# CoHDI/composable-resource-operator

Hardware: NVIDIA H100
Metric: composed-GPU probes/sec (higher is better)
Workload: dtype u64

## Files before the change

__graft_entry__.py:

```python
from __future__ import annotations

import importlib
import os
import subprocess
import sys

ROOT = os.path.dirname(os.path.abspath(__file__))
PKG = os.path.join(ROOT, "composable-resource-operator_b200")
CSRC = os.path.join(PKG, "csrc")
ORACLE = os.path.join(ROOT, "oracle")

NVCC_FLAGS = ["-gencode", "arch=compute_90a,code=sm_90a", "-O3", "-std=c++17", "-lineinfo",
              "-Xcompiler", "-fPIC"]
SOURCES = ["kernels.cu", "probe.cu", "sweeps.cu", "locate.cu", "hbm_scan.cu", "host_link.cu", "compute_probe.cu", "fullbox.cu", "c_api.cu", "harness.cu", "cluster.cu", "gojson.cpp", "identity.cpp", "reconcile.cpp", "detach.cpp",
           "fabric.cpp", "provider.cpp", "nodes.cpp", "gpus.cpp", "gpus_local.cpp", "gotypes.cpp", "env.cpp", "inventory.cpp", "nvml_ops.cpp", "pcilink.cpp",
           "compute.cpp"]


def _newer(target: str, deps) -> bool:
    if not os.path.exists(target):
        return True
    t = os.path.getmtime(target)
    return any(os.path.getmtime(d) > t for d in deps)


def _nvcc() -> str:
    for cand in (os.environ.get("NVCC"), "/usr/local/cuda/bin/nvcc", "nvcc"):
        if cand and (os.path.isabs(cand) and os.path.exists(cand) or not os.path.isabs(cand)):
            return cand
    return "nvcc"


def build_oracle() -> None:
    oso = os.path.join(ORACLE, "liboracle.so")
    osrc = os.path.join(ORACLE, "cro_oracle.c")
    if _newer(oso, [osrc]):
        subprocess.check_call(["gcc", "-O2", "-shared", "-fPIC", "-Wno-format-truncation", "-o", oso, osrc, "-lpthread"])
# ... 91 lines not shown
```

composable-resource-operator_b200/csrc/env.cpp:

```cpp
#include "env.hpp"

#include <cstdlib>
#include <cstring>

namespace cro {
namespace env {

namespace {
const Knob kKnobs[] = {
    {"CRO_FILL_WAVES", 1, 1024, 64, 0, "CTA waves of the fill kernel"},
    {"CRO_READ_WAVES", 1, 1024, 1, 0, "CTA waves of the LDG read kernels"},
    {"CRO_COPY_WAVES", 1, 1024, 128, 0, "CTA waves of the LDG copy kernel"},
    {"CRO_TMA_READ_TILE", 1024, 114688, 32768, 16, "bytes per TMA bulk load of the read ring"},
    {"CRO_TMA_READ_STAGES", 2, 16, 4, 0, "ring depth of the read kernel"},
    {"CRO_TMA_READ_THREADS", 64, 1024, 160, 32, "1 producer warp + consumer warps"},
    {"CRO_TMA_READ_CHUNK", 1, 4096, 1, 0, "tiles claimed per atomic"},
    {"CRO_TMA_READ_HINT", 0, 1, 0, 0, "1 = L2 evict_first on the bulk loads"},
    {"CRO_TMA_READ_DYN", 0, 1, 1, 0, "1 = dynamic tile claims"},
    {"CRO_TMA_READ_WAVES", 1, 64, 1, 0, "CTAs per SM slot"},
    {"CRO_TMA_COPY_TILE", 1024, 114688, 32768, 16, "bytes per TMA bulk copy of the copy ring"},
    {"CRO_TMA_COPY_STAGES", 2, 16, 4, 0, "ring depth of the copy kernel"},
    {"CRO_TMA_COPY_CHUNK", 1, 4096, 1, 0, "tiles claimed per atomic"},
    {"CRO_TMA_COPY_HINT", 0, 7, 0, 0, "bit0 evict_first loads, bit1 evict_first stores, bit2 evict_last stores"},
    {"CRO_TMA_COPY_DYN", 0, 1, 1, 0, "1 = dynamic tile claims"},
    {"CRO_TMA_COPY_WAVES", 1, 64, 1, 0, "CTAs per SM slot"},
    {"CRO_FUSED_TILE", 1024, 114688, 32768, 16, "bytes per tile of the checksumming copy"},
    {"CRO_FUSED_STAGES", 2, 16, 4, 0, "ring depth of the checksumming copy"},
    {"CRO_FUSED_CHUNK", 1, 4096, 1, 0, "tiles claimed per atomic"},
    {"CRO_FUSED_THREADS", 64, 1024, 160, 32, "1 producer warp + consumer warps of the checksumming copy"},
    {"CRO_READ_VARIANT", 0, 3, 0, 0, "CRO_READ_* forced for every sweep (0 = by size)"},
    {"CRO_COPY_VARIANT", 0, 3, 0, 0, "CRO_COPY_* forced (0 = checksumming TMA copy)"},
    {"CRO_USE_GRAPH", 0, 1, 1, 0, "replay the probe as one CUDA graph"},
    {"CRO_EXPECT_OVERLAP", 0, 1, 1, 0, "closed-form generator on a side stream under the copy sweeps"},
    {"CRO_EXPECT_CTAS", 1, 8, 1, 0, "CTAs per SM of the closed-form generator (it must leave room for the copy's CTA)"},
    {"CRO_CARVEOUT_FILL", 0, 1, 1, 0, "the fill kernel asks for the largest shared memory too (it runs beside a generator in cro_probe_all)"},
    {"CRO_P2P_UNIDIR", 0, 1, 0, 0, "measurement only: one direction per NVLink pair"},
    {"CRO_P2P_READ_VARIANT", 1, 3, 2, 0, "kernel of the NVLink read leg"},
    {"CRO_P2P_WRITE_VARIANT", 1, 3, 3, 0, "kernel of the NVLink push leg"},
    {"CRO_NVTX", 0, 1, 1, 0, "NVTX ranges around the probe phases"},
    {"CRO_HELPER_TIMEOUT_MS", 100, 600000, 30000, 0, "deadline of the out-of-process probe helper"},
};
constexpr int kN = (int)(sizeof kKnobs / sizeof kKnobs[0]);

int index_of(const char* name) {
    for (int i = 0; i < kN; ++i)
        if (strcmp(kKnobs[i].name, name) == 0) return i;
    return -1;
}
}

const Knob* table(int* n_out) {
    if (n_out) *n_out = kN;
// ... 58 lines not shown
```

composable-resource-operator_b200/csrc/fullbox.cu:

```cuda
#include <dlfcn.h>

#include "probe_internal.hpp"

namespace cro {

int upload_chase_table(cro_ctx* c, const std::vector<uint32_t>& perm, unsigned long long** table) {
    std::vector<unsigned long long> wide(perm.begin(), perm.end());
    CU_TRY(c, cudaMalloc(table, (size_t)kChaseSlots * 128));
    CU_TRY(c, cudaMemset(*table, 0, (size_t)kChaseSlots * 128));
    CU_TRY(c, cudaMemcpy2D(*table, 128, wide.data(), 8, 8, kChaseSlots, cudaMemcpyHostToDevice));
    CU_TRY(c, cudaStreamSynchronize(0));
    return CRO_OK;
}

namespace {

std::vector<std::vector<std::pair<int, int>>> one_factorisation(int n) {
    std::vector<std::vector<std::pair<int, int>>> rounds;
    if (n < 2) return rounds;
    const int m = (n % 2 == 0) ? n : n + 1;
    for (int r = 0; r < m - 1; ++r) {
        std::vector<std::pair<int, int>> pairs;
        auto add = [&](int a, int b) { if (a < n && b < n) pairs.push_back({a, b}); };
        add(m - 1, r);
// ... 179 lines not shown
    auto pair_ok = [&](int a, int b) { return a < 8 && b < 8 && c->devs[(size_t)a]->tmpl.p2p_access[b]; };
    auto push_bytes = [&](const Device* a, const Device* b) {
        return std::min<uint64_t>(std::min<uint64_t>(o.p2p_bytes, a->sweep_bytes), b->sweep_bytes);
    };
    if (p2p) {
        Range nv(c, "cro.probe_all.nvlink");
        for (size_t r = 0; r < rounds.size(); ++r) {
            std::vector<std::pair<int, int>> directed;
            for (const auto& p : rounds[r]) {
                directed.push_back({p.first, p.second});
                if (!unidir) directed.push_back({p.second, p.first});
            }
            for (const auto& pr : directed) {
                Device* a = c->devs[(size_t)pr.first].get();
                Device* b = c->devs[(size_t)pr.second].get();
                if (!pair_ok(pr.first, pr.second)) continue;
                CU_TRY(c, cudaSetDevice(a->ordinal));
                CU_TRY(c, cudaStreamWaitEvent(a->stream, b->ev_hbm_done, 0));
                if (r > 0) CU_TRY(c, cudaStreamWaitEvent(a->stream, b->ev_reread_done[r - 1], 0));
                CU_TRY(c, launch_read(a->plan, rvp, b->region, std::min<uint64_t>(o.p2p_bytes, b->sweep_bytes), imm_params(a),
                                      a->scratch, &a->d_out[kSlotP2P0 + 3 * pr.second], a->stream));
                c->launches++;
                if (push) {
                    CU_TRY(c, launch_copy(a->plan, wvp, b->region + b->sweep_bytes, a->region, push_bytes(a, b), imm_params(a),
                                          a->scratch, &a->d_out[kSlotP2P0 + 3 * pr.second + 1], a->stream));
                    c->launches++;
                }
                CU_TRY(c, cudaEventRecord(a->ev_push_done[r], a->stream));
            }
            for (const auto& pr : directed) {
                Device* a = c->devs[(size_t)pr.first].get();
                Device* b = c->devs[(size_t)pr.second].get();
                if (!pair_ok(pr.first, pr.second)) continue;
                CU_TRY(c, cudaSetDevice(b->ordinal));
                if (push) {
                    b->half_known[1] = false;
                    CU_TRY(c, cudaStreamWaitEvent(b->stream, a->ev_push_done[r], 0));
                    CU_TRY(c, launch_read(b->plan, resolve_read_variant(CRO_READ_AUTO, push_bytes(a, b), c->knobs), b->region + b->sweep_bytes,
                                          push_bytes(a, b), imm_params(b), b->scratch, &b->d_out[kSlotP2P0 + 3 * pr.first + 2], b->stream));
                    c->launches++;
                }
                CU_TRY(c, cudaEventRecord(b->ev_reread_done[r], b->stream));
            }
            if (unidir)
                for (const auto& p : rounds[r]) {
                    Device* b = c->devs[(size_t)p.second].get();
                    CU_TRY(c, cudaSetDevice(b->ordinal));
// ... 194 lines not shown
```

composable-resource-operator_b200/csrc/kernels.cu:

```cuda
#include "kernels.cuh"

#include <cuda_bf16.h>
#include <cuda_fp8.h>

#include <algorithm>
#include <cstdio>
#include <cstdlib>
#include <type_traits>

namespace cro {

__device__ __forceinline__ unsigned long long globaltimer_ns() {
    unsigned long long t;
    asm volatile("mov.u64 %0, %%globaltimer;" : "=l"(t));
    return t;
}

__device__ __forceinline__ uint4 ldg_stream(const uint4* p) {
    uint4 r;
    asm volatile("ld.global.nc.L1::no_allocate.v4.u32 {%0,%1,%2,%3}, [%4];"
                 : "=r"(r.x), "=r"(r.y), "=r"(r.z), "=r"(r.w)
                 : "l"(p));
    return r;
}

__device__ __forceinline__ uint64_t l2_policy_evict_first() {
    uint64_t p;
    asm volatile("createpolicy.fractional.L2::evict_first.b64 %0, 1.0;" : "=l"(p));
    return p;
}
__device__ __forceinline__ uint64_t l2_policy_evict_last() {
    uint64_t p;
    asm volatile("createpolicy.fractional.L2::evict_last.b64 %0, 1.0;" : "=l"(p));
    return p;
}

template <int STRIDE>
__device__ __forceinline__ void ldg128_x8(const void* p, unsigned long long (&a)[8],
                                          unsigned long long (&b)[8]) {
// ... 14 lines not shown
}
template <int STRIDE>
__device__ __forceinline__ void ldg256_x4(const void* p, uint64_t policy, unsigned long long (&w)[16]) {
    asm volatile(
        "ld.global.nc.L1::no_allocate.L2::cache_hint.v2.u64 {%0,%1}, [%16], %23;\n"
        "ld.global.nc.L1::no_allocate.L2::cache_hint.v2.u64 {%2,%3}, [%16+16], %23;\n"
        "ld.global.nc.L1::no_allocate.L2::cache_hint.v2.u64 {%4,%5}, [%16+%17], %23;\n"
        "ld.global.nc.L1::no_allocate.L2::cache_hint.v2.u64 {%6,%7}, [%16+%20], %23;\n"
        "ld.global.nc.L1::no_allocate.L2::cache_hint.v2.u64 {%8,%9}, [%16+%18], %23;\n"
        "ld.global.nc.L1::no_allocate.L2::cache_hint.v2.u64 {%10,%11}, [%16+%21], %23;\n"
        "ld.global.nc.L1::no_allocate.L2::cache_hint.v2.u64 {%12,%13}, [%16+%19], %23;\n"
        "ld.global.nc.L1::no_allocate.L2::cache_hint.v2.u64 {%14,%15}, [%16+%22], %23;\n"
        : "=l"(w[0]), "=l"(w[1]), "=l"(w[2]), "=l"(w[3]), "=l"(w[4]), "=l"(w[5]), "=l"(w[6]),
          "=l"(w[7]), "=l"(w[8]), "=l"(w[9]), "=l"(w[10]), "=l"(w[11]), "=l"(w[12]), "=l"(w[13]),
          "=l"(w[14]), "=l"(w[15])
        : "l"(p), "n"(STRIDE), "n"(2 * STRIDE), "n"(3 * STRIDE), "n"(STRIDE + 16), "n"(2 * STRIDE + 16),
          "n"(3 * STRIDE + 16), "l"(policy));
}

__device__ __forceinline__ void stg_stream(uint4* p, const uint4& v) {
    asm volatile("st.global.L1::no_allocate.v4.u32 [%0], {%1,%2,%3,%4};" ::"l"(p), "r"(v.x),
                 "r"(v.y), "r"(v.z), "r"(v.w)
                 : "memory");
}

__device__ __forceinline__ unsigned long long lo64(const uint4& v) {
    return (unsigned long long)v.x | ((unsigned long long)v.y << 32);
}
__device__ __forceinline__ unsigned long long hi64(const uint4& v) {
    return (unsigned long long)v.z | ((unsigned long long)v.w << 32);
}

__device__ __forceinline__ uint32_t smem_u32(const void* p) {
    return (uint32_t)__cvta_generic_to_shared(p);
}

__device__ __forceinline__ void mbar_init(uint64_t* bar, uint32_t count) {
    asm volatile("mbarrier.init.shared::cta.b64 [%0], %1;" ::"r"(smem_u32(bar)), "r"(count));
}
__device__ __forceinline__ void mbar_fence_init() {
    asm volatile("fence.mbarrier_init.release.cluster;" ::: "memory");
}
__device__ __forceinline__ void mbar_expect_tx(uint64_t* bar, uint32_t bytes) {
    asm volatile("mbarrier.arrive.expect_tx.shared::cta.b64 _, [%0], %1;" ::"r"(smem_u32(bar)),
                 "r"(bytes)
                 : "memory");
}
__device__ __forceinline__ void mbar_arrive(uint64_t* bar) {
    asm volatile("mbarrier.arrive.shared::cta.b64 _, [%0];" ::"r"(smem_u32(bar)) : "memory");
}
__device__ __forceinline__ void mbar_wait(uint64_t* bar, uint32_t parity) {
    asm volatile(
        "{\n"
        ".reg .pred p;\n"
        "WAIT_%=:\n"
        "mbarrier.try_wait.parity.shared::cta.b64 p, [%0], %1;\n"
        "@p bra DONE_%=;\n"
        "bra WAIT_%=;\n"
        "DONE_%=:\n"
        "}\n" ::"r"(smem_u32(bar)),
        "r"(parity)
        : "memory");
}
__device__ __forceinline__ void tma_load_1d(void* smem_dst, const void* gsrc, uint32_t bytes,
                                            uint64_t* bar) {
    asm volatile(
        "cp.async.bulk.shared::cluster.global.mbarrier::complete_tx::bytes [%0], [%1], %2, [%3];" ::
            "r"(smem_u32(smem_dst)),
        "l"(gsrc), "r"(bytes), "r"(smem_u32(bar))
        : "memory");
}
__device__ __forceinline__ void tma_store_1d(void* gdst, const void* smem_src, uint32_t bytes) {
    asm volatile("cp.async.bulk.global.shared::cta.bulk_group [%0], [%1], %2;" ::"l"(gdst),
                 "r"(smem_u32(smem_src)), "r"(bytes)
                 : "memory");
}
__device__ __forceinline__ void tma_load_1d_hint(void* smem_dst, const void* gsrc, uint32_t bytes,
                                                 uint64_t* bar, uint64_t policy) {
    asm volatile(
        "cp.async.bulk.shared::cluster.global.mbarrier::complete_tx::bytes.L2::cache_hint [%0], [%1], %2, [%3], %4;" ::
            "r"(smem_u32(smem_dst)),
        "l"(gsrc), "r"(bytes), "r"(smem_u32(bar)), "l"(policy)
        : "memory");
}
__device__ __forceinline__ void tma_store_1d_hint(void* gdst, const void* smem_src, uint32_t bytes,
                                                  uint64_t policy) {
    asm volatile("cp.async.bulk.global.shared::cta.bulk_group.L2::cache_hint [%0], [%1], %2, %3;" ::"l"(gdst),
                 "r"(smem_u32(smem_src)), "r"(bytes), "l"(policy)
                 : "memory");
}
__device__ __forceinline__ void tma_commit() {
    asm volatile("cp.async.bulk.commit_group;" ::: "memory");
}
template <int N>
__device__ __forceinline__ void tma_wait_read() {
    asm volatile("cp.async.bulk.wait_group.read %0;" ::"n"(N) : "memory");
}
__device__ __forceinline__ void tma_wait_all() {
    asm volatile("cp.async.bulk.wait_group 0;" ::: "memory");
}

struct Acc {
    unsigned long long x0 = 0, x1 = 0, s = 0, w = 0, d = 0;
};
__device__ __forceinline__ void fold2(Acc& A, unsigned long long a, unsigned long long b,
                                      unsigned long long m ) {
    const unsigned long long c = a + b;
    A.x0 ^= a;
    A.x1 ^= b;
    A.s += c;
    A.w += c * m;
    A.d += b;
}
__device__ __forceinline__ unsigned long long acc_x(const Acc& A) { return A.x0 ^ A.x1; }
__device__ __forceinline__ unsigned long long acc_w(const Acc& A) { return A.w + 2ull * A.d; }

__device__ __forceinline__ void publish(unsigned long long x, unsigned long long s, unsigned long long w,
                                        unsigned long long t_start, const SweepScratch sc,
                                        SweepOut* out, const ProbeParams& imm, const ProbeParams* pp,
                                        unsigned long long n_words) {
    __shared__ unsigned long long sx[32], ss[32], sw[32];
    __shared__ bool is_last;
#pragma unroll
    for (int o = 16; o > 0; o >>= 1) {
        x ^= __shfl_xor_sync(0xffffffffu, x, o);
        s += __shfl_xor_sync(0xffffffffu, s, o);
        w += __shfl_xor_sync(0xffffffffu, w, o);
    }
    const int warp = threadIdx.x >> 5, lane = threadIdx.x & 31;
    const int nwarps = (blockDim.x + 31) >> 5;
    if (lane == 0) { sx[warp] = x; ss[warp] = s; sw[warp] = w; }
    __syncthreads();
    if (warp == 0) {
        x = lane < nwarps ? sx[lane] : 0ull;
        s = lane < nwarps ? ss[lane] : 0ull;
        w = lane < nwarps ? sw[lane] : 0ull;
#pragma unroll
        for (int o = 16; o > 0; o >>= 1) {
            x ^= __shfl_xor_sync(0xffffffffu, x, o);
            s += __shfl_xor_sync(0xffffffffu, s, o);
            w += __shfl_xor_sync(0xffffffffu, w, o);
        }
        if (lane == 0) {
            sc.partials[blockIdx.x] = make_ulonglong4(x, s, w, 0ull);
            atomicMin(sc.tmin, t_start);
            atomicMax(sc.tmax, globaltimer_ns());
            __threadfence();
            unsigned ticket = atomicAdd(sc.counter, 1u);
            is_last = (ticket == gridDim.x - 1);
        }
    }
    __syncthreads();
    if (!is_last) return;
    __threadfence();
    x = 0; s = 0; w = 0;
    for (unsigned i = threadIdx.x; i < gridDim.x; i += blockDim.x) {
        const ulonglong2* q = reinterpret_cast<const ulonglong2*>(&sc.partials[i]);
        const ulonglong2 p0 = __ldcg(q), p1 = __ldcg(q + 1);
        x ^= p0.x; s += p0.y; w += p1.x;
    }
#pragma unroll
    for (int o = 16; o > 0; o >>= 1) {
        x ^= __shfl_xor_sync(0xffffffffu, x, o);
        s += __shfl_xor_sync(0xffffffffu, s, o);
        w += __shfl_xor_sync(0xffffffffu, w, o);
    }
    __syncthreads();
    if (lane == 0) { sx[warp] = x; ss[warp] = s; sw[warp] = w; }
    __syncthreads();
    if (threadIdx.x == 0) {
        x = 0; s = 0; w = 0;
        for (int k = 0; k < nwarps; ++k) { x ^= sx[k]; s += ss[k]; w += sw[k]; }
        out->x = x;
        out->s = s;
        out->w = w;
        out->t0 = *((volatile unsigned long long*)sc.tmin);
        out->t1 = *((volatile unsigned long long*)sc.tmax);
        out->stamp = pp ? pp->nonce : imm.nonce;
        out->n_words = n_words;
        *sc.counter = 0u;
        *sc.tmin = ~0ull;
        *sc.tmax = 0ull;
        if (sc.tile_ctr) *sc.tile_ctr = 0ull;
        __threadfence();
    }
}

__device__ __forceinline__ void publish_window(unsigned long long t_start, const SweepScratch sc, SweepOut* out,
                                               const ProbeParams& imm, const ProbeParams* pp, unsigned long long n_words) {
    atomicMin(sc.tmin, t_start);
    atomicMax(sc.tmax, globaltimer_ns());
    __threadfence();
    const unsigned ticket = atomicAdd(sc.counter, 1u);
    if (ticket == gridDim.x - 1) {
        __threadfence();
        out->x = 0; out->s = 0; out->w = 0;
        out->t0 = *((volatile unsigned long long*)sc.tmin);
        out->t1 = *((volatile unsigned long long*)sc.tmax);
        out->stamp = pp ? pp->nonce : imm.nonce;
        out->n_words = n_words;
        *sc.counter = 0u;
        *sc.tmin = ~0ull;
        *sc.tmax = 0ull;
        __threadfence();
    }
}

template <int THREADS, int UNROLL, bool INVERT = false>
// ... 307 lines not shown
    const unsigned long long t_end = globaltimer_ns();
    if (lane == 0) {
        atomicMin(&s_t0[reader ? 0 : 1], t_start);
        atomicMax(&s_t1[reader ? 0 : 1], t_end);
    }
    __syncthreads();
    if (rd.warps && s_count) {
        if (threadIdx.x == 0) atomicAdd(&lb.ctr->mismatches, s_count);
        if (threadIdx.x < 64 && s_bits[threadIdx.x]) atomicAdd(&lb.ctr->bits[threadIdx.x], s_bits[threadIdx.x]);
    }
    if (threadIdx.x == 0 && rd.warps) {
        unsigned long long x = 0, s = 0, w = 0;
        for (unsigned k = 0; k < rd.warps; ++k) { x ^= s_x[k]; s += s_s[k]; w += s_w[k]; }
        link_publish(rd, x, s, w, s_t0[0], s_t1[0], stamp);
    }
    if (threadIdx.x == 32 * rd.warps && wr.warps) link_publish(wr, 0, 0, 0, s_t0[1], s_t1[1], stamp);
}

__global__ void force_words_kernel(unsigned long long* base, unsigned long long first, unsigned long long count,
                                   unsigned long long and_mask, unsigned long long or_mask) {
    for (unsigned long long i = (unsigned long long)blockIdx.x * blockDim.x + threadIdx.x; i < count;
         i += (unsigned long long)gridDim.x * blockDim.x)
        base[first + i] = (base[first + i] & and_mask) | or_mask;
}

__device__ __forceinline__ void fold_tile(Acc& A, Acc& B, const uint4* sp, unsigned nvec, unsigned ctid,
                                          unsigned n_cons, unsigned long long v_tile) {
    unsigned i = ctid;
    for (; i + 3 * n_cons < nvec; i += 4 * n_cons) {
        const uint4 a = sp[i], b = sp[i + n_cons], c = sp[i + 2 * n_cons], d = sp[i + 3 * n_cons];
        const unsigned long long m = 4 * (v_tile + i) + 1, step = 4ull * n_cons;
        fold2(A, lo64(a), hi64(a), m);
        fold2(B, lo64(b), hi64(b), m + step);
        fold2(A, lo64(c), hi64(c), m + 2 * step);
        fold2(B, lo64(d), hi64(d), m + 3 * step);
    }
    for (; i < nvec; i += n_cons) {
        const uint4 a = sp[i];
        fold2(A, lo64(a), hi64(a), 4 * (v_tile + i) + 1);
    }
}

__global__ void __launch_bounds__(1024, 1)
hbm_read_tma_kernel(const unsigned char* __restrict__ base, unsigned long long bytes,
                    unsigned tile_bytes, unsigned stages, unsigned chunk,
                    unsigned long long* tile_ctr, const ProbeParams imm, const ProbeParams* __restrict__ pp,
                    SweepScratch sc, SweepOut* out) {
    extern __shared__ __align__(128) unsigned char ring[];
    __shared__ __align__(8) uint64_t full_bar[16];
    __shared__ __align__(8) uint64_t empty_bar[16];
    __shared__ unsigned long long tile_of[16];
    const unsigned long long t_start = globaltimer_ns();
    const int warp = threadIdx.x >> 5, lane = threadIdx.x & 31;
    const unsigned n_cons_warps = (blockDim.x >> 5) - 1;
    const unsigned long long n_tiles = (bytes + tile_bytes - 1) / tile_bytes;
    const unsigned hint = chunk >> 16;
    chunk &= 0xFFFFu;

    if (threadIdx.x == 0) {
        for (unsigned s = 0; s < stages; ++s) {
            mbar_init(&full_bar[s], 1);
            mbar_init(&empty_bar[s], n_cons_warps);
        }
// ... 823 lines not shown
        plan->read_chunk = (knob("CRO_TMA_READ_CHUNK") & 0xFFFFu) | (knob("CRO_TMA_READ_HINT") << 16);
        plan->read_dyn = knob("CRO_TMA_READ_DYN");
        const int threads = (int)knob("CRO_TMA_READ_THREADS");
        const size_t smem = (size_t)plan->read_tile * plan->read_stages;
        if ((e = plan_ring((const void*)hbm_read_tma_kernel, "CRO_TMA_READ_TILE", smem, threads)) != cudaSuccess)
            return e;
        plan->read_tma = {sms * occ * (int)knob("CRO_TMA_READ_WAVES"), threads, smem};
    }
    {
        plan->copy_tile = knob("CRO_TMA_COPY_TILE");
        plan->copy_stages = knob("CRO_TMA_COPY_STAGES");
        plan->copy_chunk = (knob("CRO_TMA_COPY_CHUNK") & 0xFFFFu) | (knob("CRO_TMA_COPY_HINT") << 16);
        plan->copy_dyn = knob("CRO_TMA_COPY_DYN");
        const size_t smem = (size_t)plan->copy_tile * plan->copy_stages;
        if ((e = plan_ring((const void*)hbm_copy_tma_kernel, "CRO_TMA_COPY_TILE", smem, 32)) != cudaSuccess)
            return e;
        plan->copy_tma = {sms * occ * (int)knob("CRO_TMA_COPY_WAVES"), 32, smem};
    }
    {
        plan->fused_tile = knob("CRO_FUSED_TILE");
        plan->fused_stages = knob("CRO_FUSED_STAGES");
        plan->fused_chunk = knob("CRO_FUSED_CHUNK") & 0xFFFFu;
        plan->fused_threads = knob("CRO_FUSED_THREADS");
        const size_t smem = (size_t)plan->fused_tile * plan->fused_stages;
        if ((e = plan_ring((const void*)hbm_copy_fused_kernel, "CRO_FUSED_TILE", smem, (int)plan->fused_threads)) != cudaSuccess)
            return e;
        plan->copy_fused = {sms * occ, (int)plan->fused_threads, smem};
    }
    for (const void* fn : {(const void*)hbm_expected_kernel, (const void*)hbm_read_tma_kernel, (const void*)hbm_copy_fused_kernel,
                           (const void*)hbm_copy_tma_kernel, (const void*)probe_finalize_kernel})
        if ((e = cudaFuncSetAttribute(fn, cudaFuncAttributePreferredSharedMemoryCarveout, cudaSharedmemCarveoutMaxShared)) != cudaSuccess)
            return e;
    if (knob("CRO_CARVEOUT_FILL"))
        if ((e = cudaFuncSetAttribute((const void*)hbm_fill_kernel<kFillThreads, kFillUnroll>, cudaFuncAttributePreferredSharedMemoryCarveout,
                                      cudaSharedmemCarveoutMaxShared)) != cudaSuccess)
            return e;
    if ((e = cudaOccupancyMaxActiveBlocksPerMultiprocessor(&occ, hbm_expected_kernel, 256, 0)) !=
        cudaSuccess)
        return e;
    plan->expect = {sms * std::min<int>(occ > 0 ? occ : 1, (int)knob("CRO_EXPECT_CTAS")), 256, 0};
    return cudaSuccess;
}

static int clamp_grid(int planned, uint64_t bytes, uint64_t tile_bytes) {
    const uint64_t tiles = (bytes + tile_bytes - 1) / tile_bytes;
    return (int)std::max<uint64_t>(1, std::min<uint64_t>((uint64_t)planned, tiles));
}

cudaError_t launch_fill(const KernelPlan& p, void* base, uint64_t bytes, const Params& pr,
                        const SweepScratch& sc, SweepOut* out, cudaStream_t st, bool invert) {
    constexpr uint64_t kTile = (uint64_t)kFillThreads * kFillUnroll * 16;
    const uint64_t tiles = (bytes + kTile - 1) / kTile;
    const int planned = (int)std::min<uint64_t>(std::max<uint64_t>((uint64_t)p.fill.grid, tiles / 4), 0x7FFFFFFFull);
// ... 31 lines not shown
    return cudaGetLastError();
}

cudaError_t launch_read(const KernelPlan& p, unsigned variant, const void* base, uint64_t bytes,
                        const Params& pr, const SweepScratch& sc, SweepOut* out, cudaStream_t st) {
    if (variant == READ_TMA) {
        hbm_read_tma_kernel<<<clamp_grid(p.read_tma.grid, bytes, p.read_tile), p.read_tma.block, p.read_tma.smem, st>>>(
            static_cast<const unsigned char*>(base), bytes, p.read_tile, p.read_stages, p.read_chunk,
            (p.read_dyn && sc.tile_ctr) ? sc.tile_ctr : nullptr, pr.imm, pr.pp, sc, out);
    } else if (variant == READ_LDG256) {
        hbm_read_ldg_kernel<kReadThreads, true><<<clamp_grid(p.read_ldg256.grid, bytes, kReadThreads * 128), p.read_ldg256.block, 0, st>>>(
            static_cast<const uint4*>(base), bytes >> 4, pr.imm, pr.pp, sc, out);
    } else {
        hbm_read_ldg_kernel<kReadThreads, false><<<clamp_grid(p.read_ldg.grid, bytes, kReadThreads * 128), p.read_ldg.block, 0, st>>>(
            static_cast<const uint4*>(base), bytes >> 4, pr.imm, pr.pp, sc, out);
    }
    return cudaGetLastError();
}

cudaError_t launch_copy(const KernelPlan& p, unsigned variant, void* dst, const void* src, uint64_t bytes,
                        const Params& pr, const SweepScratch& sc, SweepOut* out, cudaStream_t st) {
    if (variant == COPY_TMA_FUSED) {
        if (!out) return cudaErrorInvalidValue;
        hbm_copy_fused_kernel<<<clamp_grid(p.copy_fused.grid, bytes, p.fused_tile), p.copy_fused.block, p.copy_fused.smem, st>>>(
            static_cast<unsigned char*>(dst), static_cast<const unsigned char*>(src), bytes, p.fused_tile,
            p.fused_stages, p.fused_chunk, sc.tile_ctr, pr.imm, pr.pp, sc, out);
    } else if (variant == COPY_TMA) {
        unsigned long long* ctr = nullptr;
        if (p.copy_dyn && sc.tile_ctr) {
            ctr = sc.tile_ctr;
            cudaError_t e = cudaMemsetAsync(ctr, 0, sizeof(unsigned long long), st);
            if (e != cudaSuccess) return e;
        }
        hbm_copy_tma_kernel<<<clamp_grid(p.copy_tma.grid, bytes, p.copy_tile), p.copy_tma.block, p.copy_tma.smem, st>>>(
            static_cast<unsigned char*>(dst), static_cast<const unsigned char*>(src), bytes, p.copy_tile,
            p.copy_stages, p.copy_chunk, ctr, pr.imm, pr.pp, sc, out);
        if (ctr) {
            cudaError_t e = cudaMemsetAsync(ctr, 0, sizeof(unsigned long long), st);
            if (e != cudaSuccess) return e;
        }
    } else {
        hbm_copy_ldg_kernel<kCopyThreads, kCopyUnroll><<<clamp_grid(p.copy_ldg.grid, bytes, kCopyThreads * kCopyUnroll * 16), p.copy_ldg.block, 0, st>>>(
            static_cast<uint4*>(dst), static_cast<const uint4*>(src), bytes >> 4, pr.imm, pr.pp, sc, out);
    }
    return cudaGetLastError();
}
// ... 49 lines not shown
```

composable-resource-operator_b200/csrc/kernels.cuh:

```cuda
#pragma once
#include <cuda_runtime.h>
#include <stddef.h>
#include <stdint.h>

#include <string>

#include "../../include/croprobe.h"
#include "env.hpp"

namespace cro {

struct SweepOut {
    unsigned long long x;
    unsigned long long s;
    unsigned long long w;
    unsigned long long t0;
    unsigned long long t1;
    unsigned long long stamp;
    unsigned long long n_words;
    unsigned long long pad;
};
static_assert(sizeof(SweepOut) == 64 && sizeof(SweepOut) == sizeof(cro_sweep_slot), "SweepOut is one 64-byte slot");
static_assert(offsetof(SweepOut, t0) == offsetof(cro_sweep_slot, t0) && offsetof(SweepOut, stamp) == offsetof(cro_sweep_slot, stamp) &&
                  offsetof(SweepOut, n_words) == offsetof(cro_sweep_slot, n_words),
// ... 16 lines not shown
struct LaunchCfg {
    int grid;
    int block;
    size_t smem;
};

__host__ __device__ __forceinline__ unsigned long long pattern_word(unsigned long long seed,
                                                                     unsigned long long i) {
    unsigned long long z = seed + i + 0x9E3779B97F4A7C15ull;
    z = (z ^ (z >> 30)) * 0xBF58476D1CE4E5B9ull;
    z = (z ^ (z >> 27)) * 0x94D049BB133111EBull;
    return z ^ (z >> 31);
}

enum : unsigned { READ_LDG = 1, READ_TMA = 2, READ_LDG256 = 3, COPY_LDG = 1, COPY_TMA = 2, COPY_TMA_FUSED = 3 };

struct KernelPlan {
    LaunchCfg fill, read_ldg, read_ldg256, read_tma, copy_ldg, copy_tma, copy_fused, expect, locate;
    int link_grid;
    int sm_count;
    unsigned read_tile, read_stages, read_chunk, read_dyn;
    unsigned copy_tile, copy_stages, copy_chunk, copy_dyn;
    unsigned fused_tile, fused_stages, fused_chunk, fused_threads;
};
cudaError_t plan_kernels(int device, const env::Values& knobs, KernelPlan* plan, std::string* why);

struct Params {
    ProbeParams imm;
    const ProbeParams* pp;
};
cudaError_t launch_fill(const KernelPlan&, void* base, uint64_t bytes, const Params&,
                        const SweepScratch&, SweepOut* out, cudaStream_t, bool invert = false);
cudaError_t launch_read(const KernelPlan&, unsigned variant, const void* base, uint64_t bytes,
                        const Params&, const SweepScratch&, SweepOut* out, cudaStream_t);
cudaError_t launch_copy(const KernelPlan&, unsigned variant, void* dst, const void* src, uint64_t bytes,
                        const Params&, const SweepScratch&, SweepOut* out, cudaStream_t);
cudaError_t launch_expected(const KernelPlan&, uint64_t bytes, const Params&,
                            const SweepScratch&, SweepOut* out, cudaStream_t);
cudaError_t launch_xor_word(void* base, uint64_t word_index, uint64_t mask, cudaStream_t);

constexpr unsigned kLocateRecords = CRO_LOCATE_RECORDS;
constexpr unsigned kLocateGranuleShift = 21;
struct LocateRecord {
    unsigned long long word, expected, actual;
};
struct LocateCounters {
    unsigned long long mismatches;
    unsigned long long claims;
    unsigned long long bits[64];
};
struct LocateBufs {
    LocateCounters* ctr;
    LocateRecord* rec;
    unsigned long long* granules;
};
cudaError_t launch_locate(const KernelPlan&, const void* half, uint64_t bytes, uint64_t word0, uint64_t seed,
                          uint64_t invert, const LocateBufs&, const SweepScratch&, SweepOut* out, cudaStream_t);
cudaError_t launch_force_words(void* base, uint64_t first, uint64_t count, uint64_t and_mask, uint64_t or_mask,
                               int sm_count, cudaStream_t);
// ... 105 lines not shown
```

Measured before the change: 44.98.

## Add decoupled-issue TMA checksumming copy kernel with independent load and store progress

Adds a second fused copy kernel in which the producer lane polls barriers with non-blocking test_wait, issuing TMA stores as soon as tiles land and new loads as soon as slots drain, instead of an in-order ring. The default fused tile is raised to 64 KiB with a 2-stage ring, and the new kernel becomes the default while the P2P push path keeps the old one. Shared TMA and mbarrier helpers move into a common header. The aim is to keep HBM reads and writes overlapped and reduce producer stalls, at the cost of a busy-polling producer and a shallower ring.

```diff
diff --git a/__graft_entry__.py b/__graft_entry__.py
--- a/__graft_entry__.py
+++ b/__graft_entry__.py
@@ -12,7 +12,7 @@
 
 NVCC_FLAGS = ["-gencode", "arch=compute_90a,code=sm_90a", "-O3", "-std=c++17", "-lineinfo",
               "-Xcompiler", "-fPIC"]
-SOURCES = ["kernels.cu", "probe.cu", "sweeps.cu", "locate.cu", "hbm_scan.cu", "host_link.cu", "compute_probe.cu", "fullbox.cu", "c_api.cu", "harness.cu", "cluster.cu", "gojson.cpp", "identity.cpp", "reconcile.cpp", "detach.cpp",
+SOURCES = ["kernels.cu", "copy_fused.cu", "probe.cu", "sweeps.cu", "locate.cu", "hbm_scan.cu", "host_link.cu", "compute_probe.cu", "fullbox.cu", "c_api.cu", "harness.cu", "cluster.cu", "gojson.cpp", "identity.cpp", "reconcile.cpp", "detach.cpp",
            "fabric.cpp", "provider.cpp", "nodes.cpp", "gpus.cpp", "gpus_local.cpp", "gotypes.cpp", "env.cpp", "inventory.cpp", "nvml_ops.cpp", "pcilink.cpp",
            "compute.cpp"]
 
diff --git a/composable-resource-operator_b200/csrc/copy_fused.cu b/composable-resource-operator_b200/csrc/copy_fused.cu
--- /dev/null
+++ b/composable-resource-operator_b200/csrc/copy_fused.cu
@@ -0,0 +1,144 @@
+#include "kernels.cuh"
+#include "tma_ring.cuh"
+
+namespace cro {
+
+namespace {
+
+__device__ __forceinline__ bool mbar_test(uint64_t* bar, uint32_t parity) {
+    uint32_t done;
+    asm volatile(
+        "{\n"
+        ".reg .pred p;\n"
+        "mbarrier.test_wait.parity.shared::cta.b64 p, [%1], %2;\n"
+        "selp.u32 %0, 1, 0, p;\n"
+        "}\n"
+        : "=r"(done)
+        : "r"(smem_u32(bar)), "r"(parity)
+        : "memory");
+    return done != 0;
+}
+
+template <int N>
+__device__ __forceinline__ void tma_wait_read_upto(unsigned n) {
+    if constexpr (N == 0) {
+        tma_wait_read<0>();
+    } else {
+        if (n >= (unsigned)N) tma_wait_read<N>();
+        else tma_wait_read_upto<N - 1>(n);
+    }
+}
+
+}
+
+__global__ void __launch_bounds__(1024, 1)
+hbm_copy_fused2_kernel(unsigned char* __restrict__ dst, const unsigned char* __restrict__ src,
+                       unsigned long long bytes, unsigned tile_bytes, unsigned stages, unsigned chunk,
+                       unsigned long long* tile_ctr, const ProbeParams imm, const ProbeParams* __restrict__ pp,
+                       SweepScratch sc, SweepOut* out) {
+    extern __shared__ __align__(128) unsigned char ring[];
+    __shared__ __align__(8) uint64_t full_bar[16];
+    __shared__ __align__(8) uint64_t empty_bar[16];
+    __shared__ unsigned long long tile_of[16];
+    const unsigned long long t_start = globaltimer_ns();
+    const int warp = threadIdx.x >> 5, lane = threadIdx.x & 31;
+    const unsigned n_cons_warps = (blockDim.x >> 5) - 1;
+    const unsigned long long n_tiles = (bytes + tile_bytes - 1) / tile_bytes;
+    chunk &= 0xFFFFu;
+
+    if (threadIdx.x == 0) {
+        for (unsigned s = 0; s < stages; ++s) {
+            mbar_init(&full_bar[s], 1);
+            mbar_init(&empty_bar[s], n_cons_warps);
+        }
+        mbar_fence_init();
+    }
+    __syncthreads();
+
+    Acc A, B;
+    constexpr unsigned long long kEnd = ~0ull;
+    if (warp == 0) {
+        if (lane == 0) {
+            unsigned long long loads = 0, stores = 0, fetched = 0;
+            unsigned long long cur = 0, end = 0;
+            bool dry = false;
+            auto tile_len = [&](unsigned long long off) {
+                const unsigned long long left = bytes - off;
+                return left < tile_bytes ? (unsigned)left : tile_bytes;
+            };
+            while (!dry || stores < loads) {
+                while (stores < loads) {
+                    const unsigned st = (unsigned)(stores % stages);
+                    if (!mbar_test(&full_bar[st], (unsigned)((stores / stages) & 1ull))) break;
+                    const unsigned long long off = tile_of[st] * tile_bytes;
+                    tma_store_1d(dst + off, ring + (size_t)st * tile_bytes, tile_len(off));
+                    tma_commit();
+                    ++stores;
+                }
+                if (dry) continue;
+                const unsigned st = (unsigned)(loads % stages);
+                const unsigned long long use = loads / stages;
+                if (use > 0) {
+                    const unsigned long long prev = loads - stages;
+                    if (stores <= prev || !mbar_test(&empty_bar[st], (unsigned)((use - 1) & 1ull))) continue;
+                    tma_wait_read_upto<15>((unsigned)(stores - 1 - prev));
+                }
+                unsigned long long tile;
+                if (tile_ctr) {
+                    if (cur == end) { cur = atomicAdd(tile_ctr, (unsigned long long)chunk); end = cur + chunk; }
+                    tile = cur++;
+                } else {
+                    tile = blockIdx.x + fetched * (unsigned long long)gridDim.x;
+                }
+                ++fetched;
+                if (tile >= n_tiles) {
+                    dry = true;
+                    continue;
+                }
+                const unsigned long long off = tile * tile_bytes;
+                const unsigned nb = tile_len(off);
+                tile_of[st] = tile;
+                mbar_expect_tx(&full_bar[st], nb);
+                tma_load_1d(ring + (size_t)st * tile_bytes, src + off, nb, &full_bar[st]);
+                ++loads;
+            }
+            {
+                const unsigned st = (unsigned)(loads % stages);
+                const unsigned long long use = loads / stages;
+                if (use > 0) mbar_wait(&empty_bar[st], (unsigned)((use - 1) & 1ull));
+                tile_of[st] = kEnd;
+                mbar_arrive(&full_bar[st]);
+            }
+            tma_wait_all();
+        }
+    } else {
+        const unsigned ctid = threadIdx.x - 32;
+        const unsigned n_cons = n_cons_warps * 32;
+        unsigned stage = 0, phase = 0;
+        for (;;) {
+            mbar_wait(&full_bar[stage], phase);
+            const unsigned long long tile = *reinterpret_cast<volatile unsigned long long*>(&tile_of[stage]);
+            if (tile == kEnd) break;
+            const unsigned long long off = tile * tile_bytes;
+            const unsigned long long left = bytes - off;
+            const unsigned nvec = (left < tile_bytes ? (unsigned)left : tile_bytes) >> 4;
+            fold_tile(A, B, reinterpret_cast<const uint4*>(ring + (size_t)stage * tile_bytes), nvec, ctid, n_cons, off >> 4);
+            __syncwarp();
+            if (lane == 0) mbar_arrive(&empty_bar[stage]);
+            if (++stage == stages) { stage = 0; phase ^= 1u; }
+        }
+    }
+    publish(acc_x(A) ^ acc_x(B), A.s + B.s, acc_w(A) + acc_w(B), t_start, sc, out, imm, pp, bytes >> 3);
+}
+
+const void* copy_fused2_kernel() { return (const void*)hbm_copy_fused2_kernel; }
+
+cudaError_t launch_copy_fused2(const KernelPlan& p, int grid, void* dst, const void* src, uint64_t bytes, const Params& pr,
+                               const SweepScratch& sc, SweepOut* out, cudaStream_t st) {
+    hbm_copy_fused2_kernel<<<grid, p.copy_fused.block, p.copy_fused.smem, st>>>(
+        static_cast<unsigned char*>(dst), static_cast<const unsigned char*>(src), bytes, p.fused_tile, p.fused_stages,
+        p.fused_chunk, sc.tile_ctr, pr.imm, pr.pp, sc, out);
+    return cudaGetLastError();
+}
+
+}
diff --git a/composable-resource-operator_b200/csrc/env.cpp b/composable-resource-operator_b200/csrc/env.cpp
--- a/composable-resource-operator_b200/csrc/env.cpp
+++ b/composable-resource-operator_b200/csrc/env.cpp
@@ -24,10 +24,11 @@
     {"CRO_TMA_COPY_HINT", 0, 7, 0, 0, "bit0 evict_first loads, bit1 evict_first stores, bit2 evict_last stores"},
     {"CRO_TMA_COPY_DYN", 0, 1, 1, 0, "1 = dynamic tile claims"},
     {"CRO_TMA_COPY_WAVES", 1, 64, 1, 0, "CTAs per SM slot"},
-    {"CRO_FUSED_TILE", 1024, 114688, 32768, 16, "bytes per tile of the checksumming copy"},
-    {"CRO_FUSED_STAGES", 2, 16, 4, 0, "ring depth of the checksumming copy"},
+    {"CRO_FUSED_TILE", 1024, 114688, 65536, 16, "bytes per tile of the checksumming copy"},
+    {"CRO_FUSED_STAGES", 2, 16, 2, 0, "ring depth of the checksumming copy"},
     {"CRO_FUSED_CHUNK", 1, 4096, 1, 0, "tiles claimed per atomic"},
     {"CRO_FUSED_THREADS", 64, 1024, 160, 32, "1 producer warp + consumer warps of the checksumming copy"},
+    {"CRO_FUSED_KERNEL", 1, 2, 2, 0, "kernel of the checksumming copy: 1 = in-order ring, 2 = loads and stores issued apart"},
     {"CRO_READ_VARIANT", 0, 3, 0, 0, "CRO_READ_* forced for every sweep (0 = by size)"},
     {"CRO_COPY_VARIANT", 0, 3, 0, 0, "CRO_COPY_* forced (0 = checksumming TMA copy)"},
     {"CRO_USE_GRAPH", 0, 1, 1, 0, "replay the probe as one CUDA graph"},
diff --git a/composable-resource-operator_b200/csrc/fullbox.cu b/composable-resource-operator_b200/csrc/fullbox.cu
--- a/composable-resource-operator_b200/csrc/fullbox.cu
+++ b/composable-resource-operator_b200/csrc/fullbox.cu
@@ -225,7 +225,9 @@
                                       a->scratch, &a->d_out[kSlotP2P0 + 3 * pr.second], a->stream));
                 c->launches++;
                 if (push) {
-                    CU_TRY(c, launch_copy(a->plan, wvp, b->region + b->sweep_bytes, a->region, push_bytes(a, b), imm_params(a),
+                    KernelPlan push_plan = a->plan;
+                    push_plan.fused_kernel = 1;
+                    CU_TRY(c, launch_copy(push_plan, wvp, b->region + b->sweep_bytes, a->region, push_bytes(a, b), imm_params(a),
                                           a->scratch, &a->d_out[kSlotP2P0 + 3 * pr.second + 1], a->stream));
                     c->launches++;
                 }
diff --git a/composable-resource-operator_b200/csrc/kernels.cu b/composable-resource-operator_b200/csrc/kernels.cu
--- a/composable-resource-operator_b200/csrc/kernels.cu
+++ b/composable-resource-operator_b200/csrc/kernels.cu
@@ -1,4 +1,5 @@
 #include "kernels.cuh"
+#include "tma_ring.cuh"
 
 #include <cuda_bf16.h>
 #include <cuda_fp8.h>
@@ -9,12 +10,6 @@
 #include <type_traits>
 
 namespace cro {
-
-__device__ __forceinline__ unsigned long long globaltimer_ns() {
-    unsigned long long t;
-    asm volatile("mov.u64 %0, %%globaltimer;" : "=l"(t));
-    return t;
-}
 
 __device__ __forceinline__ uint4 ldg_stream(const uint4* p) {
     uint4 r;
@@ -75,168 +70,6 @@
     asm volatile("st.global.L1::no_allocate.v4.u32 [%0], {%1,%2,%3,%4};" ::"l"(p), "r"(v.x),
                  "r"(v.y), "r"(v.z), "r"(v.w)
                  : "memory");
-}
-
-__device__ __forceinline__ unsigned long long lo64(const uint4& v) {
-    return (unsigned long long)v.x | ((unsigned long long)v.y << 32);
-}
-__device__ __forceinline__ unsigned long long hi64(const uint4& v) {
-    return (unsigned long long)v.z | ((unsigned long long)v.w << 32);
-}
-
-__device__ __forceinline__ uint32_t smem_u32(const void* p) {
-    return (uint32_t)__cvta_generic_to_shared(p);
-}
-
-__device__ __forceinline__ void mbar_init(uint64_t* bar, uint32_t count) {
-    asm volatile("mbarrier.init.shared::cta.b64 [%0], %1;" ::"r"(smem_u32(bar)), "r"(count));
-}
-__device__ __forceinline__ void mbar_fence_init() {
-    asm volatile("fence.mbarrier_init.release.cluster;" ::: "memory");
-}
-__device__ __forceinline__ void mbar_expect_tx(uint64_t* bar, uint32_t bytes) {
-    asm volatile("mbarrier.arrive.expect_tx.shared::cta.b64 _, [%0], %1;" ::"r"(smem_u32(bar)),
-                 "r"(bytes)
-                 : "memory");
-}
-__device__ __forceinline__ void mbar_arrive(uint64_t* bar) {
-    asm volatile("mbarrier.arrive.shared::cta.b64 _, [%0];" ::"r"(smem_u32(bar)) : "memory");
-}
-__device__ __forceinline__ void mbar_wait(uint64_t* bar, uint32_t parity) {
-    asm volatile(
-        "{\n"
-        ".reg .pred p;\n"
-        "WAIT_%=:\n"
-        "mbarrier.try_wait.parity.shared::cta.b64 p, [%0], %1;\n"
-        "@p bra DONE_%=;\n"
-        "bra WAIT_%=;\n"
-        "DONE_%=:\n"
-        "}\n" ::"r"(smem_u32(bar)),
-        "r"(parity)
-        : "memory");
-}
-__device__ __forceinline__ void tma_load_1d(void* smem_dst, const void* gsrc, uint32_t bytes,
-                                            uint64_t* bar) {
-    asm volatile(
-        "cp.async.bulk.shared::cluster.global.mbarrier::complete_tx::bytes [%0], [%1], %2, [%3];" ::
-            "r"(smem_u32(smem_dst)),
-        "l"(gsrc), "r"(bytes), "r"(smem_u32(bar))
-        : "memory");
-}
-__device__ __forceinline__ void tma_store_1d(void* gdst, const void* smem_src, uint32_t bytes) {
-    asm volatile("cp.async.bulk.global.shared::cta.bulk_group [%0], [%1], %2;" ::"l"(gdst),
-                 "r"(smem_u32(smem_src)), "r"(bytes)
-                 : "memory");
-}
-__device__ __forceinline__ void tma_load_1d_hint(void* smem_dst, const void* gsrc, uint32_t bytes,
-                                                 uint64_t* bar, uint64_t policy) {
-    asm volatile(
-        "cp.async.bulk.shared::cluster.global.mbarrier::complete_tx::bytes.L2::cache_hint [%0], [%1], %2, [%3], %4;" ::
-            "r"(smem_u32(smem_dst)),
-        "l"(gsrc), "r"(bytes), "r"(smem_u32(bar)), "l"(policy)
-        : "memory");
-}
-__device__ __forceinline__ void tma_store_1d_hint(void* gdst, const void* smem_src, uint32_t bytes,
-                                                  uint64_t policy) {
-    asm volatile("cp.async.bulk.global.shared::cta.bulk_group.L2::cache_hint [%0], [%1], %2, %3;" ::"l"(gdst),
-                 "r"(smem_u32(smem_src)), "r"(bytes), "l"(policy)
-                 : "memory");
-}
-__device__ __forceinline__ void tma_commit() {
-    asm volatile("cp.async.bulk.commit_group;" ::: "memory");
-}
-template <int N>
-__device__ __forceinline__ void tma_wait_read() {
-    asm volatile("cp.async.bulk.wait_group.read %0;" ::"n"(N) : "memory");
-}
-__device__ __forceinline__ void tma_wait_all() {
-    asm volatile("cp.async.bulk.wait_group 0;" ::: "memory");
-}
-
-struct Acc {
-    unsigned long long x0 = 0, x1 = 0, s = 0, w = 0, d = 0;
-};
-__device__ __forceinline__ void fold2(Acc& A, unsigned long long a, unsigned long long b,
-                                      unsigned long long m ) {
-    const unsigned long long c = a + b;
-    A.x0 ^= a;
-    A.x1 ^= b;
-    A.s += c;
-    A.w += c * m;
-    A.d += b;
-}
-__device__ __forceinline__ unsigned long long acc_x(const Acc& A) { return A.x0 ^ A.x1; }
-__device__ __forceinline__ unsigned long long acc_w(const Acc& A) { return A.w + 2ull * A.d; }
-
-__device__ __forceinline__ void publish(unsigned long long x, unsigned long long s, unsigned long long w,
-                                        unsigned long long t_start, const SweepScratch sc,
-                                        SweepOut* out, const ProbeParams& imm, const ProbeParams* pp,
-                                        unsigned long long n_words) {
-    __shared__ unsigned long long sx[32], ss[32], sw[32];
-    __shared__ bool is_last;
-#pragma unroll
-    for (int o = 16; o > 0; o >>= 1) {
-        x ^= __shfl_xor_sync(0xffffffffu, x, o);
-        s += __shfl_xor_sync(0xffffffffu, s, o);
-        w += __shfl_xor_sync(0xffffffffu, w, o);
-    }
-    const int warp = threadIdx.x >> 5, lane = threadIdx.x & 31;
-    const int nwarps = (blockDim.x + 31) >> 5;
-    if (lane == 0) { sx[warp] = x; ss[warp] = s; sw[warp] = w; }
-    __syncthreads();
-    if (warp == 0) {
-        x = lane < nwarps ? sx[lane] : 0ull;
-        s = lane < nwarps ? ss[lane] : 0ull;
-        w = lane < nwarps ? sw[lane] : 0ull;
-#pragma unroll
-        for (int o = 16; o > 0; o >>= 1) {
-            x ^= __shfl_xor_sync(0xffffffffu, x, o);
-            s += __shfl_xor_sync(0xffffffffu, s, o);
-            w += __shfl_xor_sync(0xffffffffu, w, o);
-        }
-        if (lane == 0) {
-            sc.partials[blockIdx.x] = make_ulonglong4(x, s, w, 0ull);
-            atomicMin(sc.tmin, t_start);
-            atomicMax(sc.tmax, globaltimer_ns());
-            __threadfence();
-            unsigned ticket = atomicAdd(sc.counter, 1u);
-            is_last = (ticket == gridDim.x - 1);
-        }
-    }
-    __syncthreads();
-    if (!is_last) return;
-    __threadfence();
-    x = 0; s = 0; w = 0;
-    for (unsigned i = threadIdx.x; i < gridDim.x; i += blockDim.x) {
-        const ulonglong2* q = reinterpret_cast<const ulonglong2*>(&sc.partials[i]);
-        const ulonglong2 p0 = __ldcg(q), p1 = __ldcg(q + 1);
-        x ^= p0.x; s += p0.y; w += p1.x;
-    }
-#pragma unroll
-    for (int o = 16; o > 0; o >>= 1) {
-        x ^= __shfl_xor_sync(0xffffffffu, x, o);
-        s += __shfl_xor_sync(0xffffffffu, s, o);
-        w += __shfl_xor_sync(0xffffffffu, w, o);
-    }
-    __syncthreads();
-    if (lane == 0) { sx[warp] = x; ss[warp] = s; sw[warp] = w; }
-    __syncthreads();
-    if (threadIdx.x == 0) {
-        x = 0; s = 0; w = 0;
-        for (int k = 0; k < nwarps; ++k) { x ^= sx[k]; s += ss[k]; w += sw[k]; }
-        out->x = x;
-        out->s = s;
-        out->w = w;
-        out->t0 = *((volatile unsigned long long*)sc.tmin);
-        out->t1 = *((volatile unsigned long long*)sc.tmax);
-        out->stamp = pp ? pp->nonce : imm.nonce;
-        out->n_words = n_words;
-        *sc.counter = 0u;
-        *sc.tmin = ~0ull;
-        *sc.tmax = 0ull;
-        if (sc.tile_ctr) *sc.tile_ctr = 0ull;
-        __threadfence();
-    }
 }
 
 __device__ __forceinline__ void publish_window(unsigned long long t_start, const SweepScratch sc, SweepOut* out,
@@ -590,23 +423,6 @@
     for (unsigned long long i = (unsigned long long)blockIdx.x * blockDim.x + threadIdx.x; i < count;
          i += (unsigned long long)gridDim.x * blockDim.x)
         base[first + i] = (base[first + i] & and_mask) | or_mask;
-}
-
-__device__ __forceinline__ void fold_tile(Acc& A, Acc& B, const uint4* sp, unsigned nvec, unsigned ctid,
-                                          unsigned n_cons, unsigned long long v_tile) {
-    unsigned i = ctid;
-    for (; i + 3 * n_cons < nvec; i += 4 * n_cons) {
-        const uint4 a = sp[i], b = sp[i + n_cons], c = sp[i + 2 * n_cons], d = sp[i + 3 * n_cons];
-        const unsigned long long m = 4 * (v_tile + i) + 1, step = 4ull * n_cons;
-        fold2(A, lo64(a), hi64(a), m);
-        fold2(B, lo64(b), hi64(b), m + step);
-        fold2(A, lo64(c), hi64(c), m + 2 * step);
-        fold2(B, lo64(d), hi64(d), m + 3 * step);
-    }
-    for (; i < nvec; i += n_cons) {
-        const uint4 a = sp[i];
-        fold2(A, lo64(a), hi64(a), 4 * (v_tile + i) + 1);
-    }
 }
 
 __global__ void __launch_bounds__(1024, 1)
@@ -1476,13 +1292,17 @@
         plan->fused_stages = knob("CRO_FUSED_STAGES");
         plan->fused_chunk = knob("CRO_FUSED_CHUNK") & 0xFFFFu;
         plan->fused_threads = knob("CRO_FUSED_THREADS");
+        plan->fused_kernel = knob("CRO_FUSED_KERNEL");
         const size_t smem = (size_t)plan->fused_tile * plan->fused_stages;
         if ((e = plan_ring((const void*)hbm_copy_fused_kernel, "CRO_FUSED_TILE", smem, (int)plan->fused_threads)) != cudaSuccess)
             return e;
+        if (plan->fused_kernel == 2 &&
+            (e = plan_ring(copy_fused2_kernel(), "CRO_FUSED_TILE", smem, (int)plan->fused_threads)) != cudaSuccess)
+            return e;
         plan->copy_fused = {sms * occ, (int)plan->fused_threads, smem};
     }
     for (const void* fn : {(const void*)hbm_expected_kernel, (const void*)hbm_read_tma_kernel, (const void*)hbm_copy_fused_kernel,
-                           (const void*)hbm_copy_tma_kernel, (const void*)probe_finalize_kernel})
+                           copy_fused2_kernel(), (const void*)hbm_copy_tma_kernel, (const void*)probe_finalize_kernel})
         if ((e = cudaFuncSetAttribute(fn, cudaFuncAttributePreferredSharedMemoryCarveout, cudaSharedmemCarveoutMaxShared)) != cudaSuccess)
             return e;
     if (knob("CRO_CARVEOUT_FILL"))
@@ -1560,6 +1380,8 @@
                         const Params& pr, const SweepScratch& sc, SweepOut* out, cudaStream_t st) {
     if (variant == COPY_TMA_FUSED) {
         if (!out) return cudaErrorInvalidValue;
+        if (p.fused_kernel == 2)
+            return launch_copy_fused2(p, clamp_grid(p.copy_fused.grid, bytes, p.fused_tile), dst, src, bytes, pr, sc, out, st);
         hbm_copy_fused_kernel<<<clamp_grid(p.copy_fused.grid, bytes, p.fused_tile), p.copy_fused.block, p.copy_fused.smem, st>>>(
             static_cast<unsigned char*>(dst), static_cast<const unsigned char*>(src), bytes, p.fused_tile,
             p.fused_stages, p.fused_chunk, sc.tile_ctr, pr.imm, pr.pp, sc, out);
diff --git a/composable-resource-operator_b200/csrc/kernels.cuh b/composable-resource-operator_b200/csrc/kernels.cuh
--- a/composable-resource-operator_b200/csrc/kernels.cuh
+++ b/composable-resource-operator_b200/csrc/kernels.cuh
@@ -62,6 +62,7 @@
     unsigned read_tile, read_stages, read_chunk, read_dyn;
     unsigned copy_tile, copy_stages, copy_chunk, copy_dyn;
     unsigned fused_tile, fused_stages, fused_chunk, fused_threads;
+    unsigned fused_kernel;
 };
 cudaError_t plan_kernels(int device, const env::Values& knobs, KernelPlan* plan, std::string* why);
 
@@ -75,6 +76,9 @@
                         const Params&, const SweepScratch&, SweepOut* out, cudaStream_t);
 cudaError_t launch_copy(const KernelPlan&, unsigned variant, void* dst, const void* src, uint64_t bytes,
                         const Params&, const SweepScratch&, SweepOut* out, cudaStream_t);
+const void* copy_fused2_kernel();
+cudaError_t launch_copy_fused2(const KernelPlan&, int grid, void* dst, const void* src, uint64_t bytes, const Params&,
+                               const SweepScratch&, SweepOut* out, cudaStream_t);
 cudaError_t launch_expected(const KernelPlan&, uint64_t bytes, const Params&,
                             const SweepScratch&, SweepOut* out, cudaStream_t);
 cudaError_t launch_xor_word(void* base, uint64_t word_index, uint64_t mask, cudaStream_t);
diff --git a/composable-resource-operator_b200/csrc/tma_ring.cuh b/composable-resource-operator_b200/csrc/tma_ring.cuh
--- /dev/null
+++ b/composable-resource-operator_b200/csrc/tma_ring.cuh
@@ -0,0 +1,191 @@
+#pragma once
+#include "kernels.cuh"
+
+namespace cro {
+
+__device__ __forceinline__ unsigned long long globaltimer_ns() {
+    unsigned long long t;
+    asm volatile("mov.u64 %0, %%globaltimer;" : "=l"(t));
+    return t;
+}
+
+__device__ __forceinline__ unsigned long long lo64(const uint4& v) {
+    return (unsigned long long)v.x | ((unsigned long long)v.y << 32);
+}
+__device__ __forceinline__ unsigned long long hi64(const uint4& v) {
+    return (unsigned long long)v.z | ((unsigned long long)v.w << 32);
+}
+
+__device__ __forceinline__ uint32_t smem_u32(const void* p) {
+    return (uint32_t)__cvta_generic_to_shared(p);
+}
+
+__device__ __forceinline__ void mbar_init(uint64_t* bar, uint32_t count) {
+    asm volatile("mbarrier.init.shared::cta.b64 [%0], %1;" ::"r"(smem_u32(bar)), "r"(count));
+}
+__device__ __forceinline__ void mbar_fence_init() {
+    asm volatile("fence.mbarrier_init.release.cluster;" ::: "memory");
+}
+__device__ __forceinline__ void mbar_expect_tx(uint64_t* bar, uint32_t bytes) {
+    asm volatile("mbarrier.arrive.expect_tx.shared::cta.b64 _, [%0], %1;" ::"r"(smem_u32(bar)),
+                 "r"(bytes)
+                 : "memory");
+}
+__device__ __forceinline__ void mbar_arrive(uint64_t* bar) {
+    asm volatile("mbarrier.arrive.shared::cta.b64 _, [%0];" ::"r"(smem_u32(bar)) : "memory");
+}
+__device__ __forceinline__ void mbar_wait(uint64_t* bar, uint32_t parity) {
+    asm volatile(
+        "{\n"
+        ".reg .pred p;\n"
+        "WAIT_%=:\n"
+        "mbarrier.try_wait.parity.shared::cta.b64 p, [%0], %1;\n"
+        "@p bra DONE_%=;\n"
+        "bra WAIT_%=;\n"
+        "DONE_%=:\n"
+        "}\n" ::"r"(smem_u32(bar)),
+        "r"(parity)
+        : "memory");
+}
+__device__ __forceinline__ void tma_load_1d(void* smem_dst, const void* gsrc, uint32_t bytes,
+                                            uint64_t* bar) {
+    asm volatile(
+        "cp.async.bulk.shared::cluster.global.mbarrier::complete_tx::bytes [%0], [%1], %2, [%3];" ::
+            "r"(smem_u32(smem_dst)),
+        "l"(gsrc), "r"(bytes), "r"(smem_u32(bar))
+        : "memory");
+}
+__device__ __forceinline__ void tma_store_1d(void* gdst, const void* smem_src, uint32_t bytes) {
+    asm volatile("cp.async.bulk.global.shared::cta.bulk_group [%0], [%1], %2;" ::"l"(gdst),
+                 "r"(smem_u32(smem_src)), "r"(bytes)
+                 : "memory");
+}
+__device__ __forceinline__ void tma_load_1d_hint(void* smem_dst, const void* gsrc, uint32_t bytes,
+                                                 uint64_t* bar, uint64_t policy) {
+    asm volatile(
+        "cp.async.bulk.shared::cluster.global.mbarrier::complete_tx::bytes.L2::cache_hint [%0], [%1], %2, [%3], %4;" ::
+            "r"(smem_u32(smem_dst)),
+        "l"(gsrc), "r"(bytes), "r"(smem_u32(bar)), "l"(policy)
+        : "memory");
+}
+__device__ __forceinline__ void tma_store_1d_hint(void* gdst, const void* smem_src, uint32_t bytes,
+                                                  uint64_t policy) {
+    asm volatile("cp.async.bulk.global.shared::cta.bulk_group.L2::cache_hint [%0], [%1], %2, %3;" ::"l"(gdst),
+                 "r"(smem_u32(smem_src)), "r"(bytes), "l"(policy)
+                 : "memory");
+}
+__device__ __forceinline__ void tma_commit() {
+    asm volatile("cp.async.bulk.commit_group;" ::: "memory");
+}
+template <int N>
+__device__ __forceinline__ void tma_wait_read() {
+    asm volatile("cp.async.bulk.wait_group.read %0;" ::"n"(N) : "memory");
+}
+__device__ __forceinline__ void tma_wait_all() {
+    asm volatile("cp.async.bulk.wait_group 0;" ::: "memory");
+}
+
+struct Acc {
+    unsigned long long x0 = 0, x1 = 0, s = 0, w = 0, d = 0;
+};
+__device__ __forceinline__ void fold2(Acc& A, unsigned long long a, unsigned long long b,
+                                      unsigned long long m ) {
+    const unsigned long long c = a + b;
+    A.x0 ^= a;
+    A.x1 ^= b;
+    A.s += c;
+    A.w += c * m;
+    A.d += b;
+}
+__device__ __forceinline__ unsigned long long acc_x(const Acc& A) { return A.x0 ^ A.x1; }
+__device__ __forceinline__ unsigned long long acc_w(const Acc& A) { return A.w + 2ull * A.d; }
+
+__device__ __forceinline__ void publish(unsigned long long x, unsigned long long s, unsigned long long w,
+                                        unsigned long long t_start, const SweepScratch sc,
+                                        SweepOut* out, const ProbeParams& imm, const ProbeParams* pp,
+                                        unsigned long long n_words) {
+    __shared__ unsigned long long sx[32], ss[32], sw[32];
+    __shared__ bool is_last;
+#pragma unroll
+    for (int o = 16; o > 0; o >>= 1) {
+        x ^= __shfl_xor_sync(0xffffffffu, x, o);
+        s += __shfl_xor_sync(0xffffffffu, s, o);
+        w += __shfl_xor_sync(0xffffffffu, w, o);
+    }
+    const int warp = threadIdx.x >> 5, lane = threadIdx.x & 31;
+    const int nwarps = (blockDim.x + 31) >> 5;
+    if (lane == 0) { sx[warp] = x; ss[warp] = s; sw[warp] = w; }
+    __syncthreads();
+    if (warp == 0) {
+        x = lane < nwarps ? sx[lane] : 0ull;
+        s = lane < nwarps ? ss[lane] : 0ull;
+        w = lane < nwarps ? sw[lane] : 0ull;
+#pragma unroll
+        for (int o = 16; o > 0; o >>= 1) {
+            x ^= __shfl_xor_sync(0xffffffffu, x, o);
+            s += __shfl_xor_sync(0xffffffffu, s, o);
+            w += __shfl_xor_sync(0xffffffffu, w, o);
+        }
+        if (lane == 0) {
+            sc.partials[blockIdx.x] = make_ulonglong4(x, s, w, 0ull);
+            atomicMin(sc.tmin, t_start);
+            atomicMax(sc.tmax, globaltimer_ns());
+            __threadfence();
+            unsigned ticket = atomicAdd(sc.counter, 1u);
+            is_last = (ticket == gridDim.x - 1);
+        }
+    }
+    __syncthreads();
+    if (!is_last) return;
+    __threadfence();
+    x = 0; s = 0; w = 0;
+    for (unsigned i = threadIdx.x; i < gridDim.x; i += blockDim.x) {
+        const ulonglong2* q = reinterpret_cast<const ulonglong2*>(&sc.partials[i]);
+        const ulonglong2 p0 = __ldcg(q), p1 = __ldcg(q + 1);
+        x ^= p0.x; s += p0.y; w += p1.x;
+    }
+#pragma unroll
+    for (int o = 16; o > 0; o >>= 1) {
+        x ^= __shfl_xor_sync(0xffffffffu, x, o);
+        s += __shfl_xor_sync(0xffffffffu, s, o);
+        w += __shfl_xor_sync(0xffffffffu, w, o);
+    }
+    __syncthreads();
+    if (lane == 0) { sx[warp] = x; ss[warp] = s; sw[warp] = w; }
+    __syncthreads();
+    if (threadIdx.x == 0) {
+        x = 0; s = 0; w = 0;
+        for (int k = 0; k < nwarps; ++k) { x ^= sx[k]; s += ss[k]; w += sw[k]; }
+        out->x = x;
+        out->s = s;
+        out->w = w;
+        out->t0 = *((volatile unsigned long long*)sc.tmin);
+        out->t1 = *((volatile unsigned long long*)sc.tmax);
+        out->stamp = pp ? pp->nonce : imm.nonce;
+        out->n_words = n_words;
+        *sc.counter = 0u;
+        *sc.tmin = ~0ull;
+        *sc.tmax = 0ull;
+        if (sc.tile_ctr) *sc.tile_ctr = 0ull;
+        __threadfence();
+    }
+}
+
+__device__ __forceinline__ void fold_tile(Acc& A, Acc& B, const uint4* sp, unsigned nvec, unsigned ctid,
+                                          unsigned n_cons, unsigned long long v_tile) {
+    unsigned i = ctid;
+    for (; i + 3 * n_cons < nvec; i += 4 * n_cons) {
+        const uint4 a = sp[i], b = sp[i + n_cons], c = sp[i + 2 * n_cons], d = sp[i + 3 * n_cons];
+        const unsigned long long m = 4 * (v_tile + i) + 1, step = 4ull * n_cons;
+        fold2(A, lo64(a), hi64(a), m);
+        fold2(B, lo64(b), hi64(b), m + step);
+        fold2(A, lo64(c), hi64(c), m + 2 * step);
+        fold2(B, lo64(d), hi64(d), m + 3 * step);
+    }
+    for (; i < nvec; i += n_cons) {
+        const uint4 a = sp[i];
+        fold2(A, lo64(a), hi64(a), 4 * (v_tile + i) + 1);
+    }
+}
+
+}
```

New measurement: 44.96, median of 6. About the same (-0.0%).
